# MartinPippel/DAmar

Hardware: AMD Instinct MI355X
Metric: aligned base-pairs/sec (daligner block-vs-block) (higher is better)
Workload: dtype int32

## Files before the change

damar_amd/csrc/kernels/seed_merge.hip:

```cpp
#include "dev_common.h"
#include "kernels.h"

SEED_PRIO_VAR(g_merge_prio, 0)
SEED_PRIO_SETTER(damar_merge_set_prio, g_merge_prio)


__device__ __forceinline__ u32 count_below(const u32 *__restrict__ bpos, u32 jb, u32 ib, u32 bound)
{ u32 a = jb, b = ib;
  while (a < b)
    { u32 m = (a + b) >> 1;
      if (bpos[m] < bound) a = m + 1; else b = m;
    }
  return a - jb;
}


#ifndef MT_PER
#define MT_PER  4
#endif
#define MT_A    (MT_PER * 256)
#define MT_BCAP (3 * MT_A)
#define MT_HITS 4
#define MT_NBK  2048

// ... 97 lines not shown
__device__ __forceinline__ u32 self_hits(const MergeArgs &m, u32 p, u32 jb, u32 nb)
{ u32 bound;
  const int rp = m.ablk.rpbits;
  if (rp)
    { const u32 ra = p >> rp;
      bound = m.identity ? (m.comp ? (ra + 1) << rp : p) : ra << rp;
      if (m.identity && m.comp && ((ra + 1) >> (32 - rp)) != 0)
        return nb;
    }
  else if (m.identity)
    bound = m.comp ? m.ablk.boff[read_of_pos(m.ablk, p) + 1] : p;
  else
    bound = m.ablk.boff[read_of_pos(m.ablk, p)];
  return count_below(m.bpos, jb, jb + nb, bound);
}

__device__ __forceinline__ u64 block_sum_u64(u64 v, u64 *red)
{ for (int o = 32; o > 0; o >>= 1)
    { const u32 lo = (u32) __shfl_xor((int) (u32) v, o), hi = (u32) __shfl_xor((int) (u32) (v >> 32), o);
      v += ((u64) hi << 32) | lo;
    }
  __syncthreads();
  if (lane_id() == 0) red[threadIdx.x >> 6] = v;
  __syncthreads();
  return red[0] + red[1] + red[2] + red[3];
}

template <typename CodeT, bool INLDS>
__device__ __forceinline__ void merge_sweep_tile(const MergeArgs &m, const MergeTile tl, const u32 tile,
                                                 u32 *__restrict__ tcount, u32 *__restrict__ cnt, u32 *__restrict__ jbg,
                                                 unsigned long long *__restrict__ gram, u32 ngram,
                                                 CodeT *sb, u32 *loc, u32 *sjb, u32 *sw4, u64 *red)
{ const CodeT *acode = (const CodeT *) m.acode, *bcode = (const CodeT *) m.bcode;
  const int l = lane_id(), w = threadIdx.x >> 6;
  const u32 a0 = tile * (u32) MT_A, a1 = min(m.alen, a0 + (u32) MT_A), nat = a1 - a0;
  const u32 nbt = tl.b1 - tl.b0;
  const u32 e0 = threadIdx.x * MT_PER;
  const int nv = (e0 >= nat) ? 0 : (int) min((u32) MT_PER, nat - e0);

  constexpr u32 VPK = 16 / sizeof(CodeT);
  typedef CodeT VecT __attribute__((ext_vector_type(16 / sizeof(CodeT))));
  CodeT a[MT_PER];
  if (nv == MT_PER)
    {
#pragma unroll
      for (int q = 0; q < MT_PER / (int) VPK; q++)
        { const VecT v = ((const VecT *) (acode + a0 + e0))[q];
#pragma unroll
          for (int e = 0; e < (int) VPK; e++)
            a[q * VPK + e] = v[e];
        }
    }
  else
    {
#pragma unroll
      for (int k = 0; k < MT_PER; k++)
        a[k] = (k < nv) ? acode[a0 + e0 + k] : (CodeT) 0;
    }
  const u32 b0a = tl.b0 & ~(VPK - 1), sh = tl.b0 - b0a;
  const CodeT *B;
  if (INLDS)
    { const u32 nvec = (tl.b1 - b0a + VPK - 1) / VPK;
      VecT v[MT_BCAP / (int) VPK / 256 + 1];
#pragma unroll
      for (int r = 0; r < MT_BCAP / (int) VPK / 256 + 1; r++)
        { const u32 x = threadIdx.x + (u32) r * 256;
          if (x < nvec)
            { if (b0a + (x + 1) * VPK <= m.blen)
                v[r] = ((const VecT *) (bcode + b0a))[x];
              else
                {
#pragma unroll
                  for (int e = 0; e < (int) VPK; e++)
                    v[r][e] = (b0a + x * VPK + e < m.blen) ? bcode[b0a + x * VPK + e] : (CodeT) 0;
                }
            }
        }
#pragma unroll
      for (int r = 0; r < MT_BCAP / (int) VPK / 256 + 1; r++)
        { const u32 x = threadIdx.x + (u32) r * 256;
          if (x < nvec)
            ((VecT *) sb)[x] = v[r];
        }
      B = sb + sh;
    }
  else
    B = bcode + tl.b0;
  bool head0 = true;
  { CodeT prev = a[MT_PER - 1];
    if (sizeof(CodeT) == 8)
      { const u32 lo = (u32) __shfl_up((int) (u32) prev, 1), hi = (u32) __shfl_up((int) (u32) ((u64) prev >> 32), 1);
        prev = (CodeT) (((u64) hi << 32) | lo);
      }
    else
      prev = (CodeT) (u32) __shfl_up((int) (u32) prev, 1);
    if (nv > 0)
      { if (e0 == 0)
          head0 = (tl.ja == a0);
        else
          { if (l == 0) prev = acode[a0 + e0 - 1];
            head0 = (prev != a[0]);
          }
      }
  }
  __syncthreads();

  u32 jb[MT_PER], nb[MT_PER];
  { u32 p = (nv > 0) ? lower_bound_c<CodeT>(B, 0, nbt, a[0]) : 0;
#pragma unroll
    for (int k = 0; k < MT_PER; k++)
      { jb[k] = 0;  nb[k] = 0;
        if (k < nv)
          { const CodeT c = a[k];
            if (k > 0 && c == a[k - 1])
              { jb[k] = jb[k - 1];  nb[k] = nb[k - 1]; }
            else
              { int steps = 0;
                while (p < nbt && B[p] < c)
                  { p += 1;
                    if (++steps == 4) { p = lower_bound_c<CodeT>(B, p, nbt, c);  break; }
                  }
                u32 q = p;
                steps = 0;
                while (q < nbt && B[q] == c)
                  { q += 1;
                    if (++steps == 4) { q = upper_bound_c<CodeT>(B, q, nbt, c);  break; }
                  }
                jb[k] = p;  nb[k] = q - p;
                p = q;
              }
          }
      }
  }

  u32 hbits = 0;
#pragma unroll
  for (int k = 0; k < MT_PER; k++)
    { const bool h = (k >= nv) ? true : (k == 0 ? head0 : a[k] != a[k - 1]);
      hbits |= (u32) h << k;
    }
  u32 rs[MT_PER], re[MT_PER];
  bool rs_open[MT_PER];
  {
    u32 tmax = 0;
#pragma unroll
    for (int k = 0; k < MT_PER; k++)
      if ((hbits >> k) & 1) tmax = e0 + k + 1;
    u32 x = tmax;
    for (int o = 1; o < 64; o <<= 1)
      { const u32 t = (u32) __shfl_up((int) x, o);
        if (l >= o) x = max(x, t);
      }
    if (l == 63) sw4[w] = x;
    u32 carry = (u32) __shfl_up((int) x, 1);
    if (l == 0) carry = 0;
    __syncthreads();
    for (int i = 0; i < 4; i++)
      if (i < w) carry = max(carry, sw4[i]);
    __syncthreads();
#pragma unroll
    for (int k = 0; k < MT_PER; k++)
      { if ((hbits >> k) & 1) carry = e0 + k + 1;
        rs_open[k] = (carry == 0);
        rs[k] = carry ? carry - 1 : 0;
      }
    const u32 NONE = 0xffffffffu;
    u32 tmin = NONE;
#pragma unroll
    for (int k = MT_PER - 1; k >= 0; k--)
      if ((hbits >> k) & 1) tmin = e0 + k;
    x = tmin;
    for (int o = 1; o < 64; o <<= 1)
      { const u32 t = (u32) __shfl_down((int) x, o);
        if (l + o < 64) x = min(x, t);
      }
    if (l == 0) sw4[w] = x;
    u32 cb = (u32) __shfl_down((int) x, 1);
    if (l == 63) cb = NONE;
    __syncthreads();
    for (int i = 0; i < 4; i++)
      if (i > w) cb = min(cb, sw4[i]);
    __syncthreads();
#pragma unroll
    for (int k = MT_PER - 1; k >= 0; k--)
      { re[k] = (cb == NONE || cb > nat) ? nat : cb;
        if ((hbits >> k) & 1) cb = e0 + k;
      }
  }

  u32 n[MT_PER];
#pragma unroll
  for (int k = 0; k < MT_PER; k++)
    { n[k] = 0;
      if (k < nv && nb[k] > 0)
        { if (!m.self)
            { const u32 ja = rs_open[k] ? tl.ja : a0 + rs[k];
              const u32 ia = (re[k] >= nat) ? tl.ia : a0 + re[k];
              if ((u64) (ia - ja) * (u64) nb[k] < (u64) m.limit)
                n[k] = nb[k];
            }
          else
            n[k] = self_hits(m, m.apos[a0 + e0 + k], tl.b0 + jb[k], nb[k]);
        }
    }

  u64 T64;
  for (int round = 0; ; round++)
    { u32 s = 0;
      u64 s64 = 0;
#pragma unroll
      for (int k = 0; k < MT_PER; k++)
        { s += n[k];  s64 += n[k]; }
      u32 inc = (u32) wave_incl_scan_i((int) s);
      if (l == 63) sw4[w] = inc;
      __syncthreads();
      u32 ex = inc - s;
      for (int i = 0; i < 4; i++)
        if (i < w) ex += sw4[i];
      __syncthreads();
#pragma unroll
      for (int k = 0; k < MT_PER; k++)
        { loc[e0 + k] = ex;
          ex += n[k];
        }
      if (threadIdx.x == 255)
        loc[MT_A] = ex;
      T64 = block_sum_u64(s64, red);
      if (!m.self || round == 1)
        break;
      u64 xhead = 0, xtail = 0;
      if (tl.ja < a0)
        { if (threadIdx.x == 0) { sjb[0] = jb[0];  sjb[1] = nb[0]; }
          __syncthreads();
          const u32 j0 = tl.b0 + sjb[0], nn = sjb[1];
          u64 acc = 0;
          if (nn > 0)
            for (u32 i = tl.ja + threadIdx.x; i < a0; i += 256)
              acc += self_hits(m, m.apos[i], j0, nn);
          xhead = block_sum_u64(acc, red);
        }
      if (tl.ia > a1)
        { const u32 le = nat - 1;
          if (threadIdx.x == le / MT_PER)
            {
#pragma unroll
              for (int k = 0; k < MT_PER; k++)
                if (k == (int) (le % MT_PER)) { sjb[0] = jb[k];  sjb[1] = nb[k]; }
            }
          __syncthreads();
          const u32 j0 = tl.b0 + sjb[0], nn = sjb[1];
          u64 acc = 0;
          if (nn > 0)
            for (u32 i = a1 + threadIdx.x; i < tl.ia; i += 256)
              acc += self_hits(m, m.apos[i], j0, nn);
          xtail = block_sum_u64(acc, red);
        }
#pragma unroll
      for (int k = 0; k < MT_PER; k++)
        if (k < nv && nb[k] > 0)
          { u64 tot = (u64) (loc[re[k]] - loc[rs[k]]);
            if (rs_open[k]) tot += xhead;
            if (re[k] >= nat) tot += xtail;
            if (gram != NULL && ((hbits >> k) & 1) && tot < (u64) m.limit && tot < (u64) ngram)
              atomicAdd(&gram[tot], 1ull);
            if (tot >= (u64) m.limit)
              n[k] = 0;
          }
      __syncthreads();
    }

  if (!m.self && gram != NULL)
    {
#pragma unroll
      for (int k = 0; k < MT_PER; k++)
        if (k < nv && nb[k] > 0 && ((hbits >> k) & 1))
          { const u32 ia = (re[k] >= nat) ? tl.ia : a0 + re[k];
            const u64 ct = (u64) (ia - (a0 + e0 + k)) * (u64) nb[k];
            if (ct < (u64) ngram)
              atomicAdd(&gram[ct], 1ull);
          }
    }
  if (threadIdx.x == 0)
    tcount[tile] = (T64 > 0xffffffffull) ? 0xffffffffu : (u32) T64;
  typedef u32 V4 __attribute__((ext_vector_type(4)));
  if (nv == MT_PER && MT_PER == 4)
    { V4 vc, vj;
#pragma unroll
      for (int k = 0; k < 4; k++)
        { vc[k] = n[k];  vj[k] = tl.b0 + jb[k]; }
      *(V4 *) (cnt + a0 + e0) = vc;
      *(V4 *) (jbg + a0 + e0) = vj;
    }
  else
    {
#pragma unroll
      for (int k = 0; k < MT_PER; k++)
        if (k < nv)
          { cnt[a0 + e0 + k] = n[k];
            jbg[a0 + e0 + k] = tl.b0 + jb[k];
          }
    }
}

static_assert(MT_BCAP + 16 < (1 << 16), "a packed entry holds the piece-relative start and the hits in 16 bits each");
struct MergeFastArgs
{ const void *acode, *bcode;
  const u32  *apos, *bpos;
  u32 alen, blen;
  int self, identity, comp, rpbits;
};

template <typename CodeT>
__global__ __launch_bounds__(256, 8)
void merge_fast(MergeFastArgs m, MergeTile *__restrict__ tiles, u32 *__restrict__ tcount, u32 *__restrict__ cnt)
{ SEED_PRIO(g_merge_prio);
  __shared__ __attribute__((aligned(16))) CodeT sb[MT_BCAP + 16 / sizeof(CodeT)];
  __shared__ __attribute__((aligned(16))) u16 first[MT_NBK];
  __shared__ u32 wsum[4];
  __shared__ u32 deep;
  const CodeT *acode = (const CodeT *) m.acode, *bcode = (const CodeT *) m.bcode;
  const u32 tile = blockIdx.x;
  const MergeTile tl = tiles[tile];
  const u32 a0 = tile * (u32) MT_A, a1 = min(m.alen, a0 + (u32) MT_A), nat = a1 - a0;
  const u32 nbt = tl.b1 - tl.b0;
  if (nbt > MT_BCAP || (m.self && m.rpbits == 0))
    { if (threadIdx.x == 0)
        tiles[tile].pad[0] = 1;
      return;
    }
  const u32 e0 = threadIdx.x * MT_PER;
  const int nv = (e0 >= nat) ? 0 : (int) min((u32) MT_PER, nat - e0);
  const u32 sh = tl.sh, nmax = tl.pad[1];
  constexpr u32 VPK = 16 / sizeof(CodeT);
  typedef CodeT VecT __attribute__((ext_vector_type(16 / sizeof(CodeT))));
  typedef u32 V4 __attribute__((ext_vector_type(4)));

  const CodeT c0 = acode[a0];
  CodeT a[MT_PER];
  if (nv == MT_PER)
    {
#pragma unroll
      for (int q = 0; q < MT_PER / (int) VPK; q++)
        { const VecT v = ((const VecT *) (acode + a0 + e0))[q];
#pragma unroll
          for (int e = 0; e < (int) VPK; e++)
            a[q * VPK + e] = v[e];
        }
    }
  else
    {
#pragma unroll
      for (int k = 0; k < MT_PER; k++)
        a[k] = (k < nv) ? acode[a0 + e0 + k] : (CodeT) 0;
    }
  const u32 b0a = tl.b0 & ~(VPK - 1), shf = tl.b0 - b0a;
  { const u32 nvec = (tl.b1 - b0a + VPK - 1) / VPK;
    const u32 whole = (m.blen - b0a) / VPK;
    VecT v[MT_BCAP / (int) VPK / 256 + 1];
#pragma unroll
    for (int r = 0; r < MT_BCAP / (int) VPK / 256 + 1; r++)
      { const u32 x = threadIdx.x + (u32) r * 256;
        if (x < nvec)
          { if (x < whole)
              v[r] = ((const VecT *) (bcode + b0a))[x];
            else
              {
#pragma unroll
                for (int e = 0; e < (int) VPK; e++)
                  v[r][e] = (b0a + x * VPK + e < m.blen) ? bcode[b0a + x * VPK + e] : (CodeT) 0;
              }
          }
      }
    { const V4 ones = { 0xffffffffu, 0xffffffffu, 0xffffffffu, 0xffffffffu };
      ((V4 *) first)[threadIdx.x] = ones;
    }
    if (threadIdx.x == 0)
      deep = 0;
#pragma unroll
    for (int r = 0; r < MT_BCAP / (int) VPK / 256 + 1; r++)
      { const u32 x = threadIdx.x + (u32) r * 256;
        if (x < nvec)
          ((VecT *) sb)[x] = v[r];
      }
  }
  const CodeT *B = sb + shf;
  __syncthreads();
  for (u32 j = threadIdx.x; j < nbt; j += 256)
    { const u32 bk = (u32) ((B[j] - c0) >> sh);
      if (j == 0 || (u32) ((B[j - 1] - c0) >> sh) != bk)
        first[bk] = (u16) j;
    }
  __syncthreads();

  u32 jb[MT_PER], n[MT_PER];
  u32 longest = 0;
#pragma unroll
  for (int k = 0; k < MT_PER; k++)
    { jb[k] = 0;  n[k] = 0;
      if (k < nv)
        { const CodeT c = a[k];
          if (k > 0 && c == a[k - 1])
            { jb[k] = jb[k - 1];  n[k] = n[k - 1]; }
          else
            { u32 p = first[(u32) ((c - c0) >> sh)];
              if (p != 0xffffu)
                { int steps = 0;
                  while (p < nbt && B[p] < c)
                    { p += 1;
                      if (++steps == 4) { p = lower_bound_c<CodeT>(B, p, nbt, c);  break; }
                    }
                  u32 q = p;
                  steps = 0;
                  while (q < nbt && B[q] == c)
                    { q += 1;
                      if (++steps == 4) { q = upper_bound_c<CodeT>(B, q, nbt, c);  break; }
                    }
                  jb[k] = p;  n[k] = q - p;
                }
            }
          longest = max(longest, n[k]);
        }
    }
  if (longest > nmax)
    deep = 1;
  u32 sum = 0;
  if (m.self)
    { const int rp = m.rpbits;
#pragma unroll
      for (int k = 0; k < MT_PER; k++)
        if (n[k] > 0)
          { const u32 p = m.apos[a0 + e0 + k], ra = p >> rp;
            u32 bound = m.identity ? (m.comp ? (ra + 1) << rp : p) : ra << rp;
            if (!(m.identity && m.comp && ((ra + 1) >> (32 - rp)) != 0))
              n[k] = count_below(m.bpos, tl.b0 + jb[k], tl.b0 + jb[k] + n[k], bound);
          }
    }
#pragma unroll
  for (int k = 0; k < MT_PER; k++)
    sum += n[k];
  sum = (u32) wave_sum_i((int) sum);
  if (lane_id() == 0)
    wsum[threadIdx.x >> 6] = sum;
  __syncthreads();
  if (deep)
    { if (threadIdx.x == 0)
        tiles[tile].pad[0] = 1;
      return;
    }
  if (threadIdx.x == 0)
    { tcount[tile] = wsum[0] + wsum[1] + wsum[2] + wsum[3];
      tiles[tile].pad[2] = 1;
    }
  if (nv == MT_PER && MT_PER == 4)
    { V4 vc;
#pragma unroll
      for (int k = 0; k < 4; k++)
        vc[k] = (n[k] << 16) | jb[k];
      *(V4 *) (cnt + a0 + e0) = vc;
    }
  else
    {
#pragma unroll
      for (int k = 0; k < MT_PER; k++)
        if (k < nv)
          cnt[a0 + e0 + k] = (n[k] << 16) | jb[k];
    }
}

template <typename CodeT>
__global__ __launch_bounds__(256, 8)
void merge_sweep(MergeArgs m, const MergeTile *__restrict__ tiles, u32 *__restrict__ tcount, u32 *__restrict__ cnt,
                 u32 *__restrict__ jbg, unsigned long long *__restrict__ gram, u32 ngram, int only_flagged)
{ SEED_PRIO(g_merge_prio);
  __shared__ __attribute__((aligned(16))) CodeT sb[MT_BCAP + 16 / sizeof(CodeT)];
  __shared__ u32 loc[MT_A + 1];
  __shared__ u32 sjb[2];
  __shared__ u32 sw4[4];
  __shared__ u64 red[4];
  const MergeTile tl = tiles[blockIdx.x];
  if (only_flagged && tl.pad[0] == 0)
    return;
  if (tl.b1 - tl.b0 <= MT_BCAP)
    merge_sweep_tile<CodeT, true>(m, tl, blockIdx.x, tcount, cnt, jbg, gram, ngram, sb, loc, sjb, sw4, red);
  else
    merge_sweep_tile<CodeT, false>(m, tl, blockIdx.x, tcount, cnt, jbg, gram, ngram, sb, loc, sjb, sw4, red);
}

__global__ __launch_bounds__(256, 8)
void merge_emit(MergeArgs m, const MergeTile *__restrict__ tiles, const u32 *__restrict__ cnt, const u32 *__restrict__ jbg,
                const u32 *__restrict__ toff, u64 nhits, u64 *__restrict__ keys, u32 *__restrict__ vals, u32 *__restrict__ pid)
{ SEED_PRIO(g_merge_prio);
  __shared__ u32 loc[MT_A + 1];
  __shared__ u32 sjb[MT_A];
  __shared__ u32 sw4[4];
  const int l = lane_id(), w = threadIdx.x >> 6;
  const u32 tile = blockIdx.x;
  const u32 a0 = tile * (u32) MT_A, a1 = min(m.alen, a0 + (u32) MT_A), nat = a1 - a0;
  const u32 e0 = threadIdx.x * MT_PER;
  const u64 h0 = toff[tile];
  const u64 hn = (tile + 1 < gridDim.x) ? (u64) toff[tile + 1] : nhits;
  if (hn == h0)
    return;
  u32 n[MT_PER], s = 0;
  const bool packed = tiles[tile].pad[2] != 0;
  const u32 pb0 = tiles[tile].b0;
#pragma unroll
  for (int k = 0; k < MT_PER; k++)
    { const bool ok = e0 + k < nat;
      const u32 w = ok ? cnt[a0 + e0 + k] : 0;
      n[k] = packed ? w >> 16 : w;
      sjb[e0 + k] = !ok ? 0 : packed ? pb0 + (w & 0xffffu) : jbg[a0 + e0 + k];
      s += n[k];
    }
  u32 inc = (u32) wave_incl_scan_i((int) s);
  if (l == 63) sw4[w] = inc;
  __syncthreads();
  u32 ex = inc - s;
  for (int i = 0; i < 4; i++)
    if (i < w) ex += sw4[i];
#pragma unroll
  for (int k = 0; k < MT_PER; k++)
    { loc[e0 + k] = ex;
      ex += n[k];
    }
  if (threadIdx.x == 255)
    loc[MT_A] = ex;
  __syncthreads();
  const u32 T = loc[MT_A];
  for (u32 t0 = threadIdx.x; t0 < T; t0 += 256 * MT_HITS)
    { u32 ai[MT_HITS], bi[MT_HITS], pa[MT_HITS], pb[MT_HITS];
#pragma unroll
      for (int x = 0; x < MT_HITS; x++)
        { const u32 t = t0 + (u32) x * 256;
          u32 lo = 0, hi = MT_A;
          if (t < T)
            while (hi - lo > 1)
              { const u32 mid = (lo + hi) >> 1;
                if (loc[mid] <= t) lo = mid; else hi = mid;
              }
          ai[x] = a0 + lo;
          bi[x] = (t < T) ? sjb[lo] + (t - loc[lo]) : 0;
        }
#pragma unroll
      for (int x = 0; x < MT_HITS; x++)
        { const bool ok = t0 + (u32) x * 256 < T;
          pa[x] = ok ? m.apos[ai[x]] : 0;
          pb[x] = ok ? m.bpos[bi[x]] : 0;
        }
      u32 ra[MT_HITS], rb[MT_HITS], xa[MT_HITS], xb[MT_HITS];
      if (m.ablk.rpbits && m.bblk.rpbits)
        {
#pragma unroll
          for (int x = 0; x < MT_HITS; x++)
            { ra[x] = pa[x] >> m.ablk.rpbits;  xa[x] = pa[x] & ((1u << m.ablk.rpbits) - 1u);
              rb[x] = pb[x] >> m.bblk.rpbits;  xb[x] = pb[x] & ((1u << m.bblk.rpbits) - 1u);
            }
        }
      else
        {
#pragma unroll
          for (int x = 0; x < MT_HITS; x++)
            { pos_decode(m.ablk, pa[x], &ra[x], &xa[x]);
              pos_decode(m.bblk, pb[x], &rb[x], &xb[x]);
            }
        }
#pragma unroll
      for (int x = 0; x < MT_HITS; x++)
        { const u32 t = t0 + (u32) x * 256;
          const u64 h = h0 + t;
          if (t < T && h < nhits)
            { const u64 key = ((u64) rb[x] << (m.abits + m.pbits)) | ((u64) ra[x] << m.pbits) | (u64) xa[x];
              if (m.dbits)
                keys[h] = (key << m.dbits) | (u64) xb[x];
              else
                { keys[h] = key;
                  vals[h] = (u32) ((int) xa[x] - (int) xb[x]);
                }
              if (pid != NULL)
                pid[h] = (rb[x] << m.abits) | ra[x];
            }
        }
    }
}


__device__ __forceinline__ u32 count_reads_below(const MergeArgs &m, u32 jb, u32 n, u32 r)
{ if (r == 0)
    return 0;
  if (r >= m.bblk.nreads)
    return n;
  const int rp = m.bblk.rpbits;
  if (rp == 0)
    return count_below(m.bpos, jb, jb + n, m.bblk.boff[r]);
  u32 a = jb, b = jb + n;
  while (a < b)
    { const u32 mid = (a + b) >> 1;
      if ((m.bpos[mid] >> rp) < r) a = mid + 1; else b = mid;
    }
  return a - jb;
}

__global__ __launch_bounds__(256)
void merge_bread_hist(MergeArgs m, const MergeTile *__restrict__ tiles, const u32 *__restrict__ cnt, const u32 *__restrict__ jbg,
                      unsigned long long *__restrict__ hist)
{ SEED_PRIO(g_merge_prio);
  __shared__ u32 loc[MT_A + 1];
  __shared__ u32 sjb[MT_A];
  __shared__ u32 sw4[4];
  const int l = lane_id(), w = threadIdx.x >> 6;
  const u32 tile = blockIdx.x;
  const u32 a0 = tile * (u32) MT_A, a1 = min(m.alen, a0 + (u32) MT_A), nat = a1 - a0;
  const u32 e0 = threadIdx.x * MT_PER;
  u32 n[MT_PER], s = 0;
  const bool packed = tiles[tile].pad[2] != 0;
  const u32 pb0 = tiles[tile].b0;
#pragma unroll
  for (int k = 0; k < MT_PER; k++)
    { const bool ok = e0 + k < nat;
      const u32 v = ok ? cnt[a0 + e0 + k] : 0;
      n[k] = packed ? v >> 16 : v;
      sjb[e0 + k] = !ok ? 0 : packed ? pb0 + (v & 0xffffu) : jbg[a0 + e0 + k];
      s += n[k];
    }
  u32 inc = (u32) wave_incl_scan_i((int) s);
  if (l == 63) sw4[w] = inc;
  __syncthreads();
  u32 ex = inc - s;
  for (int i = 0; i < 4; i++)
    if (i < w) ex += sw4[i];
#pragma unroll
  for (int k = 0; k < MT_PER; k++)
    { loc[e0 + k] = ex;
      ex += n[k];
    }
  if (threadIdx.x == 255)
    loc[MT_A] = ex;
  __syncthreads();
  const u32 T = loc[MT_A];
  const int rp = m.bblk.rpbits;
  for (u32 t0 = 0; t0 < T; t0 += 256)
    { const u32 t = t0 + threadIdx.x;
      u32 rb = 0xffffffffu;
      if (t < T)
        { u32 lo = 0, hi = MT_A;
          while (hi - lo > 1)
            { const u32 mid = (lo + hi) >> 1;
              if (loc[mid] <= t) lo = mid; else hi = mid;
            }
          const u32 pb = m.bpos[sjb[lo] + (t - loc[lo])];
          rb = rp ? pb >> rp : read_of_pos(m.bblk, pb);
        }
      const u32 below = (u32) __shfl_up((int) rb, 1);
      const bool head = (l == 0) || below != rb;
      const u64 hm = __ballot(head);
      if (head && rb < m.bblk.nreads)
        { const u64 above = (l == 63) ? 0ull : hm >> (l + 1);
          const int len = above ? __ffsll((long long) above) : 64 - l;
          atomicAdd(&hist[rb], (unsigned long long) len);
        }
    }
}

__global__ __launch_bounds__(256)
void merge_range(MergeArgs m, const MergeTile *__restrict__ tiles, u32 *__restrict__ tcount, u32 *__restrict__ cnt,
                 u32 *__restrict__ jbg)
{ SEED_PRIO(g_merge_prio);
  __shared__ u64 red[4];
  const u32 tile = blockIdx.x;
  const u32 a0 = tile * (u32) MT_A, a1 = min(m.alen, a0 + (u32) MT_A);
  const bool packed = tiles[tile].pad[2] != 0;
  const u32 pb0 = tiles[tile].b0;
  u64 sum = 0;
  for (u32 i = a0 + threadIdx.x; i < a1; i += 256)
    { const u32 v = cnt[i];
      const u32 n = packed ? v >> 16 : v;
      if (n == 0)
        continue;
      const u32 jb = packed ? pb0 + (v & 0xffffu) : jbg[i];
      const u32 lo = count_reads_below(m, jb, n, m.b_lo), hi = count_reads_below(m, jb, n, m.b_hi);
      const u32 nn = hi > lo ? hi - lo : 0;
      if (packed)
        cnt[i] = (nn << 16) | (jb + lo - pb0);
      else
        { cnt[i] = nn;
          jbg[i] = jb + lo;
        }
      sum += nn;
    }
  const u64 T64 = block_sum_u64(sum, red);
  if (threadIdx.x == 0)
    tcount[tile] = (T64 > 0xffffffffull) ? 0xffffffffu : (u32) T64;
}


static size_t mw_tiles(u32 alen)  { return ((size_t) alen + MT_A - 1) / MT_A; }
static size_t mw_off_counts(u32 alen) { return (mw_tiles(alen) * sizeof(MergeTile) + 255) & ~(size_t) 255; }
static size_t mw_off_cnt(u32 alen)    { return mw_off_counts(alen) + (((mw_tiles(alen) + 1) * sizeof(u32) + 255) & ~(size_t) 255); }
static size_t mw_off_jb(u32 alen)     { return mw_off_cnt(alen) + (((size_t) alen * sizeof(u32) + 255) & ~(size_t) 255); }

size_t damar_merge_workspace_bytes(u32 alen)
{ return mw_off_jb(alen) + (((size_t) alen * sizeof(u32) + 255) & ~(size_t) 255); }

u32 *damar_merge_tile_counts(void *work, u32 alen) { return (u32 *) ((char *) work + mw_off_counts(alen)); }

u32 damar_merge_tiles(u32 alen) { return (u32) mw_tiles(alen); }

void damar_launch_merge_count(const MergeArgs *m, void *work, unsigned long long *gram, u32 ngram, hipStream_t st)
{ if (m->alen == 0)
    return;
  const u32 ntiles = (u32) mw_tiles(m->alen);
  MergeTile *tiles = (MergeTile *) work;
  u32 *tcount = damar_merge_tile_counts(work, m->alen);
  u32 *cnt = (u32 *) ((char *) work + mw_off_cnt(m->alen)), *jb = (u32 *) ((char *) work + mw_off_jb(m->alen));
  static int general = -1;
  if (general < 0)
    general = getenv("DAMAR_MERGE_GENERAL") != NULL;
  const bool fast = gram == NULL && !general;
  MergeFastArgs f;
  f.acode = m->acode;  f.bcode = m->bcode;  f.apos = m->apos;  f.bpos = m->bpos;  f.alen = m->alen;  f.blen = m->blen;
  f.self = m->self;  f.identity = m->identity;  f.comp = m->comp;  f.rpbits = m->ablk.rpbits;
  if (m->wide)
    { hipLaunchKernelGGL(merge_tiles<u64>, dim3((ntiles + 255) / 256), dim3(256), 0, st, *m, ntiles, tiles);
      if (fast)
        hipLaunchKernelGGL(merge_fast<u64>, dim3(ntiles), dim3(256), 0, st, f, tiles, tcount, cnt);
      hipLaunchKernelGGL(merge_sweep<u64>, dim3(ntiles), dim3(256), 0, st, *m, tiles, tcount, cnt, jb, gram, ngram, fast ? 1 : 0);
    }
  else
    { hipLaunchKernelGGL(merge_tiles<u32>, dim3((ntiles + 255) / 256), dim3(256), 0, st, *m, ntiles, tiles);
      if (fast)
        hipLaunchKernelGGL(merge_fast<u32>, dim3(ntiles), dim3(256), 0, st, f, tiles, tcount, cnt);
      hipLaunchKernelGGL(merge_sweep<u32>, dim3(ntiles), dim3(256), 0, st, *m, tiles, tcount, cnt, jb, gram, ngram, fast ? 1 : 0);
    }
}

void damar_launch_merge_emit(const MergeArgs *m, void *work, u64 nhits, u64 *keys, u32 *vals, u32 *pid, hipStream_t st)
{ if (nhits == 0)
    return;
  const u32 ntiles = (u32) mw_tiles(m->alen);
  const u32 *toff = damar_merge_tile_counts(work, m->alen);
  const u32 *cnt = (const u32 *) ((char *) work + mw_off_cnt(m->alen)), *jb = (const u32 *) ((char *) work + mw_off_jb(m->alen));
  hipLaunchKernelGGL(merge_emit, dim3(ntiles), dim3(256), 0, st, *m, (const MergeTile *) work, cnt, jb, toff, nhits, keys, vals, pid);
}

void damar_launch_merge_bread_hist(const MergeArgs *m, void *work, unsigned long long *hist, hipStream_t st)
{ if (m->alen == 0)
    return;
  const u32 ntiles = (u32) mw_tiles(m->alen);
  const u32 *cnt = (const u32 *) ((char *) work + mw_off_cnt(m->alen)), *jb = (const u32 *) ((char *) work + mw_off_jb(m->alen));
  hipLaunchKernelGGL(merge_bread_hist, dim3(ntiles), dim3(256), 0, st, *m, (const MergeTile *) work, cnt, jb, hist);
}

void damar_launch_merge_range(const MergeArgs *m, void *work, hipStream_t st)
{ if (m->alen == 0)
    return;
  const u32 ntiles = (u32) mw_tiles(m->alen);
  u32 *tcount = damar_merge_tile_counts(work, m->alen);
  u32 *cnt = (u32 *) ((char *) work + mw_off_cnt(m->alen)), *jb = (u32 *) ((char *) work + mw_off_jb(m->alen));
  hipLaunchKernelGGL(merge_range, dim3(ntiles), dim3(256), 0, st, *m, (const MergeTile *) work, tcount, cnt, jb);
}

#define SCREEN_MAX   48
#define SCREEN_PANEL 50000
template <typename K>
__global__ __launch_bounds__(64)
void slice_ends(const K *__restrict__ keys, u64 nhits, u64 off, u64 gtotal, int bshift, int nshift, u64 *__restrict__ send)
{ const int nthr = 1 << nshift, t = threadIdx.x;
  if (t >= nthr)
    return;
  const u64 g = (t == nthr - 1) ? gtotal : (gtotal * (u64) (t + 1)) >> nshift;
  u64 e;
  if (g <= off)
    e = 0;
  else if (g > off + nhits)
    e = ~0ull;
  else
    { e = g - off;
      u64 d = keys[e - 1] >> bshift, a = e, b = nhits;
      while (a < b)
        { u64 mid = (a + b) >> 1;
          if ((keys[mid] >> bshift) == d) a = mid + 1; else b = mid;
        }
      e = a;
    }
  send[t] = e;
}

#define PH_ROUNDS (DAMAR_SCAN_TILE / 256)
template <typename K>
__global__ __launch_bounds__(256)
void pair_heads_mark(const K *__restrict__ keys, u64 nhits, int pbits, int minhit, int nshift,
                     const u64 *__restrict__ send, u64 *__restrict__ bits, u32 *__restrict__ tcount)
{ SEED_PRIO(g_merge_prio);
  __shared__ u32 wsum[4];
  const int nthr = nshift < 0 ? 0 : 1 << nshift;
  const int l = lane_id(), w = threadIdx.x >> 6;
  const u64 base = (u64) blockIdx.x * DAMAR_SCAN_TILE;
  u32 mine = 0;
  u64 e0 = ~0ull, e1 = ~0ull;
  for (int t = 0; t < nthr; t++)
    { const u64 e = send[t];
      if (e > base)
        { e0 = e;
          if (t + 1 < nthr)
            e1 = send[t + 1];
          break;
        }
    }
  for (int r0 = 0; r0 < PH_ROUNDS; r0 += 4)
    { K k0[4], km[4], kp[4];
#pragma unroll
      for (int q = 0; q < 4; q++)
        { const u64 i = base + (u64) (r0 + q) * 256u + threadIdx.x;
          const u64 ic = i < nhits ? i : nhits - 1;
          const u64 ip = ic + (u64) (minhit - 1);
          k0[q] = keys[ic];
          km[q] = keys[ic > 0 ? ic - 1 : 0];
          kp[q] = keys[ip < nhits ? ip : nhits - 1];
        }
#pragma unroll
      for (int q = 0; q < 4; q++)
        { const int r = r0 + q;
          const u64 i = base + (u64) r * 256u + threadIdx.x;
          bool f = false;
          if (i < nhits)
            { const K pr = k0[q] >> pbits;
              if ((i == 0 || (km[q] >> pbits) != pr) && i + (u64) (minhit - 1) < nhits && (kp[q] >> pbits) == pr)
                { f = true;
                  if (i < e0)
                    { if (i + (u64) minhit >= e0) f = false; }
                  else if (i < e1)
                    { if (i + (u64) minhit >= e1) f = false; }
                  else
                    for (int t = 0; t < nthr; t++)
                      { u64 e = send[t];
                        if (i < e)
                          { if (i + (u64) minhit >= e) f = false;
                            break;
                          }
                      }
                }
            }
          const u64 m = __ballot(f);
          if (l == 0)
            { bits[(base >> 6) + (u64) r * 4 + w] = m;
              mine += (u32) __popcll(m);
            }
        }
    }
  if (l == 0) wsum[w] = mine;
  __syncthreads();
  if (threadIdx.x == 0)
    tcount[blockIdx.x] = wsum[0] + wsum[1] + wsum[2] + wsum[3];
}

__global__ __launch_bounds__(64)
void pair_heads_expand(const u64 *__restrict__ bits, const u32 *__restrict__ toff, u32 *__restrict__ heads)
{ const u64 wi = (u64) blockIdx.x * 64u + threadIdx.x;
  u64 m = bits[wi];
  const int c = __popcll(m);
  u32 o = toff[blockIdx.x] + (u32) (wave_incl_scan_i(c) - c);
  const u32 first = (u32) (wi << 6);
  while (m)
    { const int b = __ffsll((long long) m) - 1;
      m &= m - 1;
      heads[o++] = first + (u32) b;
    }
}

template <typename K>
static void pair_heads_impl(const K *keys, u64 nhits, u64 off, u64 gtotal, int pbits, int abits, int minhit, int nshift,
                            u64 *send , u64 *bits, void *scan_work, u64 *total_dev,
                            u32 *heads, hipStream_t st)
{ if (nhits == 0)
    { HIP_CHECK(hipMemsetAsync(total_dev, 0, sizeof(u64), st));
      return;
    }
  if (nshift > 6)
    nshift = 6;
  const u32 ntiles = (u32) ((nhits + DAMAR_SCAN_TILE - 1) / DAMAR_SCAN_TILE);
  u32 *tcount = (u32 *) scan_work;
  if (nshift >= 0)
    hipLaunchKernelGGL(slice_ends<K>, dim3(1), dim3(64), 0, st, keys, nhits, off, gtotal, abits + pbits, nshift, send);
  hipLaunchKernelGGL(pair_heads_mark<K>, dim3(ntiles), dim3(256), 0, st, keys, nhits, pbits, minhit, nshift, send, bits, tcount);
  damar_scan_tile_counts(tcount, ntiles, total_dev, st);
  hipLaunchKernelGGL(pair_heads_expand, dim3(ntiles), dim3(64), 0, st, bits, tcount, heads);
}

void damar_launch_pair_heads(const u64 *keys, u64 nhits, u64 off, u64 gtotal, int pbits, int abits, int minhit, int nshift,
                             u64 *send, u64 *bits, void *scan_work, u64 *total_dev, u32 *heads, hipStream_t st)
{ pair_heads_impl<u64>(keys, nhits, off, gtotal, pbits, abits, minhit, nshift, send, bits, scan_work, total_dev, heads, st);
}


void damar_launch_pair_heads_ids(const u32 *pids, u64 nhits, u64 off, u64 gtotal, int abits, int minhit, int nshift,
                                 u64 *send, u64 *bits, void *scan_work, u64 *total_dev, u32 *heads, hipStream_t st)
{ pair_heads_impl<u32>(pids, nhits, off, gtotal, 0, abits, minhit, nshift, send, bits, scan_work, total_dev, heads, st);
}

__global__ __launch_bounds__(256)
void pair_bitmap_set(const u32 *__restrict__ pids, const u32 *__restrict__ heads, u32 nheads, int abits, u32 b_lo, u32 b_hi,
                     u32 *__restrict__ bitmap)
{ const u32 t = blockIdx.x * 256u + threadIdx.x;
  if (t >= nheads)
    return;
  const u32 p = pids[heads[t]], rb = p >> abits;
  if (rb < b_lo || rb >= b_hi)
    return;
  atomicOr(&bitmap[p >> 5], 1u << (p & 31));
}

void damar_launch_pair_bitmap(const u32 *pids, const u32 *heads, u32 nheads, int abits, u32 b_lo, u32 b_hi, u32 *bitmap,
                              hipStream_t st)
{ if (nheads == 0)
    return;
  hipLaunchKernelGGL(pair_bitmap_set, dim3((nheads + 255) / 256), dim3(256), 0, st, pids, heads, nheads, abits, b_lo, b_hi, bitmap);
}

__global__ __launch_bounds__(256)
void seed_cut_count(const u64 *__restrict__ keys, u64 nhits, int pbits, const u32 *__restrict__ bitmap, u32 *__restrict__ tcount)
{ __shared__ u32 wsum[4];
  const int l = lane_id(), w = threadIdx.x >> 6;
  const u64 base = (u64) blockIdx.x * DAMAR_SCAN_TILE;
  u32 mine = 0;
  for (int r = 0; r < PH_ROUNDS; r++)
    { const u64 i = base + (u64) r * 256u + threadIdx.x;
      bool f = false;
      if (i < nhits)
        { const u32 p = (u32) (keys[i] >> pbits);
          f = (bitmap[p >> 5] >> (p & 31)) & 1;
        }
      mine += (u32) __popcll(__ballot(f));
    }
  if (l == 0) wsum[w] = mine;
  __syncthreads();
  if (threadIdx.x == 0)
    tcount[blockIdx.x] = wsum[0] + wsum[1] + wsum[2] + wsum[3];
}

__global__ __launch_bounds__(256)
void seed_cut_scatter(const u64 *__restrict__ keys, const u32 *__restrict__ vals, u64 nhits, int pbits,
                      const u32 *__restrict__ bitmap, const u32 *__restrict__ toff, u64 *__restrict__ okeys, u32 *__restrict__ ovals)
{ __shared__ u32 wsum[PH_ROUNDS][4];
  const int l = lane_id(), w = threadIdx.x >> 6;
  const u64 base = (u64) blockIdx.x * DAMAR_SCAN_TILE;
  u64 key[PH_ROUNDS];
  u64 mask[PH_ROUNDS];
  for (int r = 0; r < PH_ROUNDS; r++)
    { const u64 i = base + (u64) r * 256u + threadIdx.x;
      bool f = false;
      key[r] = 0;
      if (i < nhits)
        { key[r] = keys[i];
          const u32 p = (u32) (key[r] >> pbits);
          f = (bitmap[p >> 5] >> (p & 31)) & 1;
        }
      mask[r] = __ballot(f);
      if (l == 0) wsum[r][w] = (u32) __popcll(mask[r]);
    }
  __syncthreads();
  u32 o = toff[blockIdx.x];
  for (int r = 0; r < PH_ROUNDS; r++)
    { u32 before = 0;
      for (int x = 0; x < 4; x++)
        { const u32 c = wsum[r][x];
          if (x < w) before += c;
        }
      const u64 i = base + (u64) r * 256u + threadIdx.x;
      if ((mask[r] >> l) & 1)
        { const u32 g = o + before + (u32) __popcll(mask[r] & lanes_below(l));
          okeys[g] = key[r];
          if (vals != NULL)
            ovals[g] = vals[i];
        }
      o += wsum[r][0] + wsum[r][1] + wsum[r][2] + wsum[r][3];
    }
}

void damar_launch_seed_cut_count(const u64 *keys, u64 nhits, int pbits, const u32 *bitmap, u32 *tcount, u64 *total_dev,
                                 hipStream_t st)
{ const u32 ntiles = (u32) ((nhits + DAMAR_SCAN_TILE - 1) / DAMAR_SCAN_TILE);
  hipLaunchKernelGGL(seed_cut_count, dim3(ntiles), dim3(256), 0, st, keys, nhits, pbits, bitmap, tcount);
  damar_scan_tile_counts(tcount, ntiles, total_dev, st);
}

void damar_launch_seed_cut_scatter(const u64 *keys, const u32 *vals, u64 nhits, int pbits, const u32 *bitmap,
                                   const u32 *toff, u64 *okeys, u32 *ovals, hipStream_t st)
{ const u32 ntiles = (u32) ((nhits + DAMAR_SCAN_TILE - 1) / DAMAR_SCAN_TILE);
  hipLaunchKernelGGL(seed_cut_scatter, dim3(ntiles), dim3(256), 0, st, keys, vals, nhits, pbits, bitmap, toff, okeys, ovals);
}

__global__ __launch_bounds__(256)
void pair_screen(const u64 *__restrict__ keys, const u32 *__restrict__ vals, u64 nhits, int pbits, int dbits,
                 const u32 *__restrict__ heads, u32 nheads, int minhit, int binshift, int kmer, int hitmin,
                 int abits, u32 b_lo, u32 b_hi, u32 *__restrict__ keep)
{ SEED_PRIO(g_merge_prio);
  u32 t = blockIdx.x * 256u + threadIdx.x;
  if (t >= nheads)
    return;
  const u64 i = heads[t];
  const u64 pmask = (1ull << pbits) - 1;
  pbits += dbits;
  const u64 pr = keys[i] >> pbits;
  u32 f = 1;
  int n = minhit;
  { const u32 rb = (u32) (pr >> abits);
    if (rb < b_lo || rb >= b_hi)
      { keep[t] = 0;
        return;
      }
  }
  while (n <= SCREEN_MAX && i + (u64) n < nhits && (keys[i + (u64) n] >> pbits) == pr)
    n += 1;
  if (n <= SCREEN_MAX && (int) ((keys[i + (u64) (n - 1)] >> dbits) & pmask) <= SCREEN_PANEL)
    { bool ok = false;
      int dlast = 0x7fffffff;
      for (int x = 0; x < n && !ok; x++)
        { const int dx = seed_diag(keys[i + (u64) x], vals, i + (u64) x, pmask, dbits) >> binshift;
          if (dx == dlast)
            continue;
          dlast = dx;
          int s0 = 0, s1 = 0, p0 = 0, p1 = 0;
          for (int y = 0; y < n; y++)
            { const u64 ky = keys[i + (u64) y];
              const int dy = seed_diag(ky, vals, i + (u64) y, pmask, dbits) >> binshift;
              const int ap = (int) ((ky >> dbits) & pmask);
              if (dy == dx)
                { s0 += (ap - p0 >= kmer) ? kmer : ap - p0;  p0 = ap; }
              else if (dy == dx + 1)
                { s1 += (ap - p1 >= kmer) ? kmer : ap - p1;  p1 = ap; }
            }
          ok = s0 + s1 >= hitmin;
        }
      if (!ok)
        f = 0;
    }
  keep[t] = f;
}

void damar_launch_pair_screen(const u64 *keys, const u32 *vals, u64 nhits, int pbits, int dbits, const u32 *heads, u32 nheads,
                              int minhit, int binshift, int kmer, int hitmin, int abits, u32 b_lo, u32 b_hi,
                              u32 *keep, hipStream_t st)
{ if (nheads == 0)
    return;
  hipLaunchKernelGGL(pair_screen, dim3((nheads + 255) / 256), dim3(256), 0, st, keys, vals, nhits, pbits, dbits, heads, nheads,
// ... 660 lines not shown
```

Measured before the change: 54.26 billion.

## Run merge count and emit kernels over multi-tile runs with prefetch of next tile

Adds merge_fast_run and merge_emit_run kernels. Each block processes MT_RUN consecutive tiles and prefetches the next tile's A codes, B codes and counts into registers while it works on the current tile, using double-buffered shared state. The aim is to hide global load latency and cut per-block launch and setup overhead. The cost is fewer blocks (less parallelism), more register pressure from the register-held B vectors, and the emit path also specialises a cheaper rpbits decode. It is enabled by default and can be disabled with DAMAR_MERGE_RUN=0.

New measurement: 54.21 billion, median of 3. No clear change (-0.1%).

```diff
diff --git a/damar_amd/csrc/kernels/seed_merge.hip b/damar_amd/csrc/kernels/seed_merge.hip
--- a/damar_amd/csrc/kernels/seed_merge.hip
+++ b/damar_amd/csrc/kernels/seed_merge.hip
@@ -423,6 +423,7 @@
     }
 }
 
+static_assert(MT_PER == 4, "the run kernels move an entry's four words as one vector");
 static_assert(MT_BCAP + 16 < (1 << 16), "a packed entry holds the piece-relative start and the hits in 16 bits each");
 struct MergeFastArgs
 { const void *acode, *bcode;
@@ -588,6 +589,225 @@
     }
 }
 
+#ifndef MT_RUN
+#define MT_RUN 8
+#endif
+#define MT_NBV(CodeT) (MT_BCAP / (16 / (int) sizeof(CodeT)) / 256 + 1)
+
+template <typename CodeT> struct MtVec { typedef CodeT type __attribute__((ext_vector_type(16 / sizeof(CodeT)))); };
+
+struct MtDesc { u32 b0, b1, sh, nmax; };
+__device__ __forceinline__ MtDesc mt_desc(const MergeTile *__restrict__ rt, u32 tile)
+{ MtDesc d;
+  d.b0 = rt[tile].b0;  d.b1 = rt[tile].b1;  d.sh = rt[tile].sh;  d.nmax = rt[tile].pad[1];
+  return d;
+}
+
+template <typename CodeT>
+__device__ __forceinline__ void mt_fetch(const MergeFastArgs &m, u32 tile, const MtDesc &d, CodeT (&a)[MT_PER],
+                                         typename MtVec<CodeT>::type (&v)[MT_NBV(CodeT)])
+{ typedef typename MtVec<CodeT>::type VecT;
+  constexpr u32 VPK = 16 / sizeof(CodeT);
+  const CodeT *acode = (const CodeT *) m.acode, *bcode = (const CodeT *) m.bcode;
+  const u32 a0 = tile * (u32) MT_A, nat = min(m.alen, a0 + (u32) MT_A) - a0;
+  const u32 e0 = threadIdx.x * MT_PER;
+  const int nv = (e0 >= nat) ? 0 : (int) min((u32) MT_PER, nat - e0);
+  if (nv == MT_PER)
+    {
+#pragma unroll
+      for (int q = 0; q < MT_PER / (int) VPK; q++)
+        { const VecT x = ((const VecT *) (acode + a0 + e0))[q];
+#pragma unroll
+          for (int e = 0; e < (int) VPK; e++)
+            a[q * VPK + e] = x[e];
+        }
+    }
+  else
+    {
+#pragma unroll
+      for (int k = 0; k < MT_PER; k++)
+        a[k] = (k < nv) ? acode[a0 + e0 + k] : (CodeT) 0;
+    }
+  const u32 b0a = d.b0 & ~(VPK - 1);
+  const u32 nvec = (d.b1 - b0a + VPK - 1) / VPK;
+  const u32 whole = (m.blen - b0a) / VPK;
+#pragma unroll
+  for (int r = 0; r < MT_NBV(CodeT); r++)
+    { const u32 x = threadIdx.x + (u32) r * 256;
+      if (x < nvec && x < whole)
+        v[r] = ((const VecT *) (bcode + b0a))[x];
+    }
+}
+
+template <typename CodeT>
+__device__ __forceinline__ void mt_stage(const MergeFastArgs &m, const MtDesc &d, CodeT *sb,
+                                         const typename MtVec<CodeT>::type (&v)[MT_NBV(CodeT)])
+{ typedef typename MtVec<CodeT>::type VecT;
+  constexpr u32 VPK = 16 / sizeof(CodeT);
+  const u32 b0a = d.b0 & ~(VPK - 1);
+  const u32 nvec = (d.b1 - b0a + VPK - 1) / VPK;
+  const u32 whole = (m.blen - b0a) / VPK;
+#pragma unroll
+  for (int r = 0; r < MT_NBV(CodeT); r++)
+    { const u32 x = threadIdx.x + (u32) r * 256;
+      if (x < nvec && x < whole)
+        ((VecT *) sb)[x] = v[r];
+    }
+  if (whole < nvec && threadIdx.x < VPK)
+    { const u32 j = whole * VPK + threadIdx.x;
+      sb[j] = (b0a + j < m.blen) ? ((const CodeT *) m.bcode)[b0a + j] : (CodeT) 0;
+    }
+}
+
+template <typename CodeT, bool SELF>
+__global__ __launch_bounds__(256, 8)
+void merge_fast_run(MergeFastArgs m, MergeTile *__restrict__ tiles, const MergeTile *__restrict__ rtiles, u32 ntiles,
+                    u32 *__restrict__ tcount, u32 *__restrict__ cnt)
+{ SEED_PRIO(g_merge_prio);
+  __shared__ __attribute__((aligned(16))) CodeT sb[MT_BCAP + 16 / sizeof(CodeT)];
+  __shared__ __attribute__((aligned(16))) u16 first[MT_NBK];
+  __shared__ u32 wsum[4];
+  __shared__ u32 deep[2];
+  __shared__ CodeT sc0;
+  typedef typename MtVec<CodeT>::type VecT;
+  typedef u32 V4 __attribute__((ext_vector_type(4)));
+  constexpr u32 VPK = 16 / sizeof(CodeT);
+  const u32 tile0 = blockIdx.x * (u32) MT_RUN, tend = min(ntiles, tile0 + (u32) MT_RUN);
+  const bool never = SELF && m.rpbits == 0;
+  const u32 e0 = threadIdx.x * MT_PER;
+
+  MtDesc tl = mt_desc(rtiles, tile0);
+  bool fits = !never && tl.b1 - tl.b0 <= MT_BCAP;
+  CodeT a[MT_PER];
+  VecT v[MT_NBV(CodeT)];
+  if (fits)
+    mt_fetch<CodeT>(m, tile0, tl, a, v);
+  if (threadIdx.x == 0)
+    deep[0] = deep[1] = 0;
+  u32 ph = 0;
+
+  for (u32 tile = tile0; tile < tend; tile++)
+    { const bool more = tile + 1 < tend;
+      MtDesc tln = tl;
+      if (more)
+        tln = mt_desc(rtiles, tile + 1);
+      const bool fitsn = more && !never && tln.b1 - tln.b0 <= MT_BCAP;
+      CodeT an[MT_PER];
+      const u32 a0 = tile * (u32) MT_A, nat = min(m.alen, a0 + (u32) MT_A) - a0;
+      const int nv = (e0 >= nat) ? 0 : (int) min((u32) MT_PER, nat - e0);
+      const u32 nbt = tl.b1 - tl.b0, sh = tl.sh, nmax = tl.nmax;
+      const u32 b0a = tl.b0 & ~(VPK - 1), shf = tl.b0 - b0a;
+      const CodeT *B = sb + shf;
+      if (!fits)
+        { if (threadIdx.x == 0)
+            tiles[tile].pad[0] = 1;
+        }
+      else
+        {
+          { const V4 ones = { 0xffffffffu, 0xffffffffu, 0xffffffffu, 0xffffffffu };
+            ((V4 *) first)[threadIdx.x] = ones;
+            if (threadIdx.x == 0)
+              sc0 = a[0];
+            mt_stage<CodeT>(m, tl, sb, v);
+          }
+          __syncthreads();
+        }
+      if (fitsn)
+        mt_fetch<CodeT>(m, tile + 1, tln, an, v);
+      if (fits)
+        { if (threadIdx.x == 0)
+            deep[ph ^ 1] = 0;
+          const CodeT c0 = sc0;
+          for (u32 j = threadIdx.x; j < nbt; j += 256)
+            { const u32 bk = (u32) ((B[j] - c0) >> sh);
+              if (j == 0 || (u32) ((B[j - 1] - c0) >> sh) != bk)
+                first[bk] = (u16) j;
+            }
+          __syncthreads();
+
+          u32 jb[MT_PER], n[MT_PER];
+          u32 longest = 0;
+#pragma unroll
+          for (int k = 0; k < MT_PER; k++)
+            { jb[k] = 0;  n[k] = 0;
+              if (k < nv)
+                { const CodeT c = a[k];
+                  if (k > 0 && c == a[k - 1])
+                    { jb[k] = jb[k - 1];  n[k] = n[k - 1]; }
+                  else
+                    { u32 p = first[(u32) ((c - c0) >> sh)];
+                      if (p != 0xffffu)
+                        { int steps = 0;
+                          while (p < nbt && B[p] < c)
+                            { p += 1;
+                              if (++steps == 4) { p = lower_bound_c<CodeT>(B, p, nbt, c);  break; }
+                            }
+                          u32 q = p;
+                          steps = 0;
+                          while (q < nbt && B[q] == c)
+                            { q += 1;
+                              if (++steps == 4) { q = upper_bound_c<CodeT>(B, q, nbt, c);  break; }
+                            }
+                          jb[k] = p;  n[k] = q - p;
+                        }
+                    }
+                  longest = max(longest, n[k]);
+                }
+            }
+          if (longest > nmax)
+            deep[ph] = 1;
+          u32 sum = 0;
+          if (SELF)
+            { const int rp = m.rpbits;
+#pragma unroll
+              for (int k = 0; k < MT_PER; k++)
+                if (n[k] > 0)
+                  { const u32 p = m.apos[a0 + e0 + k], ra = p >> rp;
+                    u32 bound = m.identity ? (m.comp ? (ra + 1) << rp : p) : ra << rp;
+                    if (!(m.identity && m.comp && ((ra + 1) >> (32 - rp)) != 0))
+                      n[k] = count_below(m.bpos, tl.b0 + jb[k], tl.b0 + jb[k] + n[k], bound);
+                  }
+            }
+#pragma unroll
+          for (int k = 0; k < MT_PER; k++)
+            sum += n[k];
+          sum = (u32) wave_sum_i((int) sum);
+          if (lane_id() == 0)
+            wsum[threadIdx.x >> 6] = sum;
+          __syncthreads();
+          if (deep[ph])
+            { if (threadIdx.x == 0)
+                tiles[tile].pad[0] = 1;
+            }
+          else
+            { if (threadIdx.x == 0)
+                { tcount[tile] = wsum[0] + wsum[1] + wsum[2] + wsum[3];
+                  tiles[tile].pad[2] = 1;
+                }
+              if (nv == MT_PER && MT_PER == 4)
+                { V4 vc;
+#pragma unroll
+                  for (int k = 0; k < 4; k++)
+                    vc[k] = (n[k] << 16) | jb[k];
+                  *(V4 *) (cnt + a0 + e0) = vc;
+                }
+              else
+                {
+#pragma unroll
+                  for (int k = 0; k < MT_PER; k++)
+                    if (k < nv)
+                      cnt[a0 + e0 + k] = (n[k] << 16) | jb[k];
+                }
+            }
+          ph ^= 1;
+        }
+      tl = tln;  fits = fitsn;
+#pragma unroll
+      for (int k = 0; k < MT_PER; k++)
+        a[k] = an[k];
+    }
+}
+
 template <typename CodeT>
 __global__ __launch_bounds__(256, 8)
 void merge_sweep(MergeArgs m, const MergeTile *__restrict__ tiles, u32 *__restrict__ tcount, u32 *__restrict__ cnt,
@@ -701,6 +921,147 @@
                 pid[h] = (rb[x] << m.abits) | ra[x];
             }
         }
+    }
+}
+
+struct MtEmitNext { u64 hn;  u32 h0, pb0;  bool packed; };
+__device__ __forceinline__ MtEmitNext mt_emit_desc(const MergeTile *__restrict__ tiles, const u32 *__restrict__ toff,
+                                                    u32 tile, u32 ntiles, u64 nhits)
+{ MtEmitNext d;
+  d.h0 = toff[tile];
+  d.hn = (tile + 1 < ntiles) ? (u64) toff[tile + 1] : nhits;
+  d.packed = tiles[tile].pad[2] != 0;
+  d.pb0 = tiles[tile].b0;
+  return d;
+}
+__device__ __forceinline__ void mt_emit_fetch(u32 alen, const u32 *__restrict__ cnt, u32 tile, u32 (&c)[MT_PER])
+{ typedef u32 V4 __attribute__((ext_vector_type(4)));
+  const u32 a0 = tile * (u32) MT_A, nat = min(alen, a0 + (u32) MT_A) - a0;
+  const u32 e0 = threadIdx.x * MT_PER;
+  if (e0 < nat)
+    { const V4 x = *(const V4 *) (cnt + a0 + e0);
+#pragma unroll
+      for (int k = 0; k < 4; k++)
+        c[k] = x[k];
+    }
+}
+
+template <bool RP>
+__global__ __launch_bounds__(256, 8)
+void merge_emit_run(MergeArgs m, const MergeTile *__restrict__ tiles, u32 ntiles, const u32 *__restrict__ cnt,
+                    const u32 *__restrict__ jbg, const u32 *__restrict__ toff, u64 nhits, u64 *__restrict__ keys,
+                    u32 *__restrict__ vals, u32 *__restrict__ pid)
+{ SEED_PRIO(g_merge_prio);
+  __shared__ u32 loc2[2][MT_A + 1];
+  __shared__ u32 sjb2[2][MT_A];
+  __shared__ u32 sw42[2][4];
+  const int l = lane_id(), w = threadIdx.x >> 6;
+  const u32 tile0 = blockIdx.x * (u32) MT_RUN, tend = min(ntiles, tile0 + (u32) MT_RUN);
+  const u32 e0 = threadIdx.x * MT_PER;
+  MtEmitNext d = mt_emit_desc(tiles, toff, tile0, ntiles, nhits), dn = d;
+  u32 c[MT_PER];
+  if (d.hn != (u64) d.h0)
+    mt_emit_fetch(m.alen, cnt, tile0, c);
+  u32 ph = 0;
+  for (u32 tile = tile0; tile < tend; tile++)
+    { const bool more = tile + 1 < tend;
+      if (more)
+        dn = mt_emit_desc(tiles, toff, tile + 1, ntiles, nhits);
+      const bool hitsn = more && dn.hn != (u64) dn.h0;
+      u32 cn[MT_PER];
+      const bool hits = d.hn != (u64) d.h0;
+      u32 *loc = loc2[ph], *sjb = sjb2[ph], *sw4 = sw42[ph];
+      const u32 a0 = tile * (u32) MT_A, nat = min(m.alen, a0 + (u32) MT_A) - a0;
+      const u64 h0 = d.h0;
+      if (hits)
+        { u32 n[MT_PER], s = 0;
+#pragma unroll
+          for (int k = 0; k < MT_PER; k++)
+            { const bool ok = e0 + k < nat;
+              const u32 x = ok ? c[k] : 0;
+              n[k] = d.packed ? x >> 16 : x;
+              sjb[e0 + k] = !ok ? 0 : d.packed ? d.pb0 + (x & 0xffffu) : jbg[a0 + e0 + k];
+              s += n[k];
+            }
+          u32 inc = (u32) wave_incl_scan_i((int) s);
+          if (l == 63) sw4[w] = inc;
+          __syncthreads();
+          u32 ex = inc - s;
+          for (int i = 0; i < 4; i++)
+            if (i < w) ex += sw4[i];
+#pragma unroll
+          for (int k = 0; k < MT_PER; k++)
+            { loc[e0 + k] = ex;
+              ex += n[k];
+            }
+          if (threadIdx.x == 255)
+            loc[MT_A] = ex;
+          __syncthreads();
+        }
+      if (hitsn)
+        mt_emit_fetch(m.alen, cnt, tile + 1, cn);
+      if (hits)
+        { const u32 T = loc[MT_A];
+          for (u32 t0 = threadIdx.x; t0 < T; t0 += 256 * MT_HITS)
+            { u32 ai[MT_HITS], bi[MT_HITS], pa[MT_HITS], pb[MT_HITS];
+#pragma unroll
+              for (int x = 0; x < MT_HITS; x++)
+                { const u32 t = t0 + (u32) x * 256;
+                  u32 lo = 0, hi = MT_A;
+                  if (t < T)
+                    while (hi - lo > 1)
+                      { const u32 mid = (lo + hi) >> 1;
+                        if (loc[mid] <= t) lo = mid; else hi = mid;
+                      }
+                  ai[x] = a0 + lo;
+                  bi[x] = (t < T) ? sjb[lo] + (t - loc[lo]) : 0;
+                }
+#pragma unroll
+              for (int x = 0; x < MT_HITS; x++)
+                { const bool ok = t0 + (u32) x * 256 < T;
+                  pa[x] = ok ? m.apos[ai[x]] : 0;
+                  pb[x] = ok ? m.bpos[bi[x]] : 0;
+                }
+              u32 ra[MT_HITS], rb[MT_HITS], xa[MT_HITS], xb[MT_HITS];
+              if (RP)
+                {
+#pragma unroll
+                  for (int x = 0; x < MT_HITS; x++)
+                    { ra[x] = pa[x] >> m.ablk.rpbits;  xa[x] = pa[x] & ((1u << m.ablk.rpbits) - 1u);
+                      rb[x] = pb[x] >> m.bblk.rpbits;  xb[x] = pb[x] & ((1u << m.bblk.rpbits) - 1u);
+                    }
+                }
+              else
+                {
+#pragma unroll
+                  for (int x = 0; x < MT_HITS; x++)
+                    { pos_decode(m.ablk, pa[x], &ra[x], &xa[x]);
+                      pos_decode(m.bblk, pb[x], &rb[x], &xb[x]);
+                    }
+                }
+#pragma unroll
+              for (int x = 0; x < MT_HITS; x++)
+                { const u32 t = t0 + (u32) x * 256;
+                  const u64 h = h0 + t;
+                  if (t < T && h < nhits)
+                    { const u64 key = ((u64) rb[x] << (m.abits + m.pbits)) | ((u64) ra[x] << m.pbits) | (u64) xa[x];
+                      if (m.dbits)
+                        keys[h] = (key << m.dbits) | (u64) xb[x];
+                      else
+                        { keys[h] = key;
+                          vals[h] = (u32) ((int) xa[x] - (int) xb[x]);
+                        }
+                      if (pid != NULL)
+                        pid[h] = (rb[x] << m.abits) | ra[x];
+                    }
+                }
+            }
+          ph ^= 1;
+        }
+      d = dn;
+#pragma unroll
+      for (int k = 0; k < MT_PER; k++)
+        c[k] = cn[k];
     }
 }
 
@@ -826,6 +1187,8 @@
 
 u32 damar_merge_tiles(u32 alen) { return (u32) mw_tiles(alen); }
 
+static int g_merge_run = 1;
+
 void damar_launch_merge_count(const MergeArgs *m, void *work, unsigned long long *gram, u32 ngram, hipStream_t st)
 { if (m->alen == 0)
     return;
@@ -835,20 +1198,36 @@
   u32 *cnt = (u32 *) ((char *) work + mw_off_cnt(m->alen)), *jb = (u32 *) ((char *) work + mw_off_jb(m->alen));
   static int general = -1;
   if (general < 0)
-    general = getenv("DAMAR_MERGE_GENERAL") != NULL;
+    { general = getenv("DAMAR_MERGE_GENERAL") != NULL;
+      const char *e = getenv("DAMAR_MERGE_RUN");
+      g_merge_run = !(e != NULL && e[0] == '0');
+    }
+  const u32 nruns = (ntiles + MT_RUN - 1) / MT_RUN;
   const bool fast = gram == NULL && !general;
   MergeFastArgs f;
   f.acode = m->acode;  f.bcode = m->bcode;  f.apos = m->apos;  f.bpos = m->bpos;  f.alen = m->alen;  f.blen = m->blen;
   f.self = m->self;  f.identity = m->identity;  f.comp = m->comp;  f.rpbits = m->ablk.rpbits;
   if (m->wide)
     { hipLaunchKernelGGL(merge_tiles<u64>, dim3((ntiles + 255) / 256), dim3(256), 0, st, *m, ntiles, tiles);
-      if (fast)
+      if (fast && g_merge_run)
+        { if (f.self)
+            hipLaunchKernelGGL((merge_fast_run<u64, true>), dim3(nruns), dim3(256), 0, st, f, tiles, (const MergeTile *) tiles, ntiles, tcount, cnt);
+          else
+            hipLaunchKernelGGL((merge_fast_run<u64, false>), dim3(nruns), dim3(256), 0, st, f, tiles, (const MergeTile *) tiles, ntiles, tcount, cnt);
+        }
+      else if (fast)
         hipLaunchKernelGGL(merge_fast<u64>, dim3(ntiles), dim3(256), 0, st, f, tiles, tcount, cnt);
       hipLaunchKernelGGL(merge_sweep<u64>, dim3(ntiles), dim3(256), 0, st, *m, tiles, tcount, cnt, jb, gram, ngram, fast ? 1 : 0);
     }
   else
     { hipLaunchKernelGGL(merge_tiles<u32>, dim3((ntiles + 255) / 256), dim3(256), 0, st, *m, ntiles, tiles);
-      if (fast)
+      if (fast && g_merge_run)
+        { if (f.self)
+            hipLaunchKernelGGL((merge_fast_run<u32, true>), dim3(nruns), dim3(256), 0, st, f, tiles, (const MergeTile *) tiles, ntiles, tcount, cnt);
+          else
+            hipLaunchKernelGGL((merge_fast_run<u32, false>), dim3(nruns), dim3(256), 0, st, f, tiles, (const MergeTile *) tiles, ntiles, tcount, cnt);
+        }
+      else if (fast)
         hipLaunchKernelGGL(merge_fast<u32>, dim3(ntiles), dim3(256), 0, st, f, tiles, tcount, cnt);
       hipLaunchKernelGGL(merge_sweep<u32>, dim3(ntiles), dim3(256), 0, st, *m, tiles, tcount, cnt, jb, gram, ngram, fast ? 1 : 0);
     }
@@ -860,7 +1239,15 @@
   const u32 ntiles = (u32) mw_tiles(m->alen);
   const u32 *toff = damar_merge_tile_counts(work, m->alen);
   const u32 *cnt = (const u32 *) ((char *) work + mw_off_cnt(m->alen)), *jb = (const u32 *) ((char *) work + mw_off_jb(m->alen));
-  hipLaunchKernelGGL(merge_emit, dim3(ntiles), dim3(256), 0, st, *m, (const MergeTile *) work, cnt, jb, toff, nhits, keys, vals, pid);
+  if (g_merge_run)
+    { const dim3 grid((ntiles + MT_RUN - 1) / MT_RUN);
+      if (m->ablk.rpbits && m->bblk.rpbits)
+        hipLaunchKernelGGL(merge_emit_run<true>, grid, dim3(256), 0, st, *m, (const MergeTile *) work, ntiles, cnt, jb, toff, nhits, keys, vals, pid);
+      else
+        hipLaunchKernelGGL(merge_emit_run<false>, grid, dim3(256), 0, st, *m, (const MergeTile *) work, ntiles, cnt, jb, toff, nhits, keys, vals, pid);
+    }
+  else
+    hipLaunchKernelGGL(merge_emit, dim3(ntiles), dim3(256), 0, st, *m, (const MergeTile *) work, cnt, jb, toff, nhits, keys, vals, pid);
 }
 
 void damar_launch_merge_bread_hist(const MergeArgs *m, void *work, unsigned long long *hist, hipStream_t st)
```
